# HKUST-Aerial-Robotics/FIESTA

Hardware: NVIDIA H100
Metric: esdf_voxel_updates_per_s (higher is better)
Workload: dtype int32+f64

## Files before the change

fiesta_b200/csrc/fb_exact.cu:

```cuda
#include <cub/cub.cuh>
#include <stdio.h>
#include <stdlib.h>
#include <algorithm>
#include <chrono>
#include "fb_common.cuh"
#include "fb_exact.h"

#define XNONE 0xffffffffu
#define XMB_NONE 0xffffffffffffffffull

__device__ __forceinline__ void x_coords(const FbGeom &g, uint32_t ii, int &x, int &y, int &z) {
  z = ii % (unsigned)g.pz; const unsigned xy = ii / (unsigned)g.pz; y = xy % (unsigned)g.gy; x = xy / (unsigned)g.gy;
}
__device__ __forceinline__ unsigned x_d2(int x, int y, int z, uint32_t c) {
  int ox, oy, oz; fb_unpack(c, ox, oy, oz); ox -= x; oy -= y; oz -= z;
  return (unsigned)(ox * ox + oy * oy + oz * oz);
}
__device__ __forceinline__ unsigned x_dist_of(int x, int y, int z, uint32_t c) { return c < 2u ? 0xffffffffu : x_d2(x, y, z, c); }

__global__ void k_x_flag_exist(const uint32_t *list, unsigned n, const double *occ, double l_occ, uint8_t *flags, int want) {
  const unsigned i = blockIdx.x * blockDim.x + threadIdx.x;
  if (i < n) flags[i] = ((occ[list[i]] > l_occ) ? 1 : 0) == want;
}
__global__ void k_x_apply_seed(FbGeom g, const uint32_t *E, unsigned n, uint32_t *cobs, unsigned long long *LS, unsigned long long t0) {
// ... 61 lines not shown

static inline unsigned nblk(size_t n, unsigned t = 256) { return (unsigned)((n + t - 1) / t); }

static int x_select(FbExact *X, const uint32_t *in, const uint8_t *flags, uint32_t *out, unsigned n, unsigned *count, cudaStream_t s) {
  *count = 0;
  if (n == 0) return FIESTA_OK;
  size_t bytes = 0;
  CK(cub::DeviceSelect::Flagged(nullptr, bytes, in, flags, out, X->d_count.p, (int)n, s));
  CK(X->cub_tmp.grow(bytes, s));
  CK(cub::DeviceSelect::Flagged(X->cub_tmp.p, bytes, in, flags, out, X->d_count.p, (int)n, s));
  CK(cudaMemcpyAsync(X->h_count, X->d_count, 4, cudaMemcpyDeviceToHost, s));
  CK(cudaStreamSynchronize(s));
  *count = *X->h_count;
  return FIESTA_OK;
}
static int x_sort_pairs(FbExact *X, const unsigned long long *kin, unsigned long long *kout, const uint32_t *vin, uint32_t *vout, unsigned n, cudaStream_t s,
                        int key_bits = 64) {
  size_t bytes = 0;
  CK(cub::DeviceRadixSort::SortPairs(nullptr, bytes, kin, kout, vin, vout, (int)n, 0, key_bits, s));
  CK(X->cub_tmp.grow(bytes, s));
  CK(cub::DeviceRadixSort::SortPairs(X->cub_tmp.p, bytes, kin, kout, vin, vout, (int)n, 0, key_bits, s));
  return FIESTA_OK;
}
int fb_exact_init(FbExact *X, const FbGeom &g, int device, cudaStream_t s) {
  const size_t P = (size_t)g.ptotal;
  CK(fb_xrelax_init());
  X->relax_blocks = fb_xrelax_blocks(device);
  if (X->relax_blocks <= 0 || X->relax_blocks > FB_X_MAX_BLOCKS) { fb_set_error("exact mode init: k_x_relax does not fit on this device"); return FIESTA_ERR_CUDA; }
  CK(X->MB.alloc(P)); CK(X->LS.alloc(P)); CK(X->tkey.alloc(P));
  CK(X->touched.alloc(P));
  CK(X->SUM.alloc(P)); CK(X->SUMg.alloc(P)); CK(cudaMemsetAsync(X->SUMg, 0, P * 4, s));
  CK(X->emask.alloc(P));
  CK(X->wstamp.alloc(P)); CK(cudaMemsetAsync(X->wstamp, 0, P * 4, s));
  for (int k = 0; k < 3; ++k) { CK(X->W[k].alloc(P)); CK(X->F[k].alloc(P)); }
  for (int k = 0; k < 2; ++k) CK(X->E[k].alloc(P));
  X->dense_min = 16384u;
  if (const char *e = getenv("FIESTA_X_DENSE")) { long v = atol(e); if (v >= 0 && v <= (1 << 24)) X->dense_min = (unsigned)v; }
  X->small_max = FB_X_SMALL_DEFAULT;
  if (const char *e = getenv("FIESTA_X_SMALL")) { long v = atol(e); if (v >= 0 && v <= 65536) X->small_max = (unsigned)v; }
  CK(X->slotc.alloc(((size_t)X->small_max + 1) * 32));
  const size_t c0 = P / 8 > (1u << 20) ? P / 8 : (1u << 20);
  for (FbDevBuf<unsigned long long> *b : {&X->k1, &X->k2, &X->k1b, &X->k2b}) CK(b->grow(c0, s));
  for (FbDevBuf<uint32_t> *b : {&X->dv, &X->idx[0], &X->idx[1], &X->deps, &X->nc[0], &X->nc[1], &X->sel}) CK(b->grow(c0, s));
  CK(X->flags.grow(c0, s)); CK(X->flags2.grow(c0, s));
  CK(X->cub_tmp.grow(c0 * 16 + (64u << 20), s));
  CK(X->d_ctl.alloc(1)); CK(cudaMemsetAsync(X->d_ctl, 0, sizeof(FbXCtl), s));
  CK(X->h_ctl.alloc(1));
  CK(X->d_count.alloc(4)); CK(X->d_flag.alloc(4));
  CK(X->h_count.alloc(4));
  CK(cudaMemsetAsync(X->d_count, 0, 16, s)); CK(cudaMemsetAsync(X->d_flag, 0, 16, s));
  k_x_fill64<<<FB_SMS * 8, 256, 0, s>>>(X->MB, P, XMB_NONE);
  CK(cudaMemsetAsync(X->tkey, 0, P * 8, s));
  CK(cudaMemsetAsync(X->LS, 0, P * 8, s));
  X->tclock = 1; X->key_base = 0; X->key_epoch = 1; X->key_hi = 1ull << FB_KEY_BITS; X->gen_id = 0; X->wclock = 0; X->sclock = 0;
  CK(cudaGetLastError());
  return FIESTA_OK;
}

int fb_exact_queue_crossings(FbExact *X, const unsigned long long *ins_key, const uint32_t *ins_vox, const unsigned long long *del_key,
                             const uint32_t *del_vox, FbDevBuf<uint32_t> &ins, unsigned *n_ins, FbDevBuf<uint32_t> &del, unsigned *n_del,
                             cudaStream_t s, int *launches) {
  int r;
  CK(cudaMemcpyAsync(X->h_count, X->d_count, 8, cudaMemcpyDeviceToHost, s));
  CK(cudaStreamSynchronize(s));
  const unsigned ni = X->h_count[0], nd = X->h_count[1];
  CK(ins.grow((size_t)*n_ins + ni, s, *n_ins));
  CK(del.grow((size_t)*n_del + nd, s, *n_del));
  CK(X->k1b.grow(ni > nd ? ni : nd, s));
  if (ni) { if ((r = x_sort_pairs(X, ins_key, X->k1b, ins_vox, ins + *n_ins, ni, s, FB_KEY_BITS))) return r; *n_ins += ni; *launches += 1; }
  if (nd) { if ((r = x_sort_pairs(X, del_key, X->k1b, del_vox, del + *n_del, nd, s, FB_KEY_BITS))) return r; *n_del += nd; *launches += 1; }
// ... 77 lines not shown
        } else {
          k_x_iota<<<nblk(ndep), 256, 0, s>>>(X->idx[0], ndep);
          if ((r = x_sort_pairs(X, X->k2, X->k2b, X->idx[0], X->idx[1], ndep, s))) return r;
          k_x_gather64<<<nblk(ndep), 256, 0, s>>>(X->k1, X->idx[1], ndep, X->k1b);
          if ((r = x_sort_pairs(X, X->k1b, X->k2b, X->idx[1], X->idx[0], ndep, s))) return r;
          k_x_gather32<<<nblk(ndep), 256, 0, s>>>(X->dv, X->idx[0], ndep, X->deps);
          *launches += 5;
        }
        CK(X->flags2.grow(ndep, s));
        k_x_set_ord<<<nblk(ndep), 256, 0, s>>>(X->deps, ndep, scratch, X->nc[0], X->flags2);
        *launches += 1;
        ndep_run = ndep; ls_deps = X->tclock;
        X->tclock += ndep;
      }
    }
  }
  st->generations = 0;
  if (xdbg) { cudaStreamSynchronize(s); fprintf(stderr, "[x] seeds+deletes %.2f ms (reseed rounds %u, dependants %u)\n", ms(t_begin, now()), st->reseed_rounds, st->dependants); }
  if (nE || ndep_run) {
    if (xdbg && !X->d_dbg) CK(X->d_dbg.alloc(FB_X_DBG_WORDS));
    if (xdbg) CK(cudaMemsetAsync(X->d_dbg, 0, FB_X_DBG_WORDS * 8, s));
    if (X->sclock > 0xf0000000u) { CK(cudaMemsetAsync(X->SUMg, 0, P * 4, s)); X->sclock = 0; }
    if (X->gen_id > 0xf0000000u) X->gen_id = 0;
    if (X->wclock > 0xf0000000u) { CK(cudaMemsetAsync(X->wstamp, 0, P * 4, s)); X->wclock = 0; }
    FbXCtl *h = X->h_ctl;
    memset(h, 0, sizeof(*h));
    h->gen_id = X->gen_id; h->wclock = X->wclock; h->tclock = X->tclock; h->sclock = X->sclock;
    CK(cudaMemcpyAsync(X->d_ctl, h, sizeof(FbXCtl), cudaMemcpyHostToDevice, s));
    CK(fb_xrelax_launch(X, g, cobs, nE, X->deps, ndep_run, scratch, X->nc[0], X->flags2, occbits, ls_deps, xdbg ? X->d_dbg.p : nullptr, s));
    if (ndep_run) k_x_unset<<<nblk(ndep_run), 256, 0, s>>>(X->deps, ndep_run, scratch);
    CK(cudaMemcpyAsync(h, X->d_ctl, sizeof(FbXCtl), cudaMemcpyDeviceToHost, s));
    CK(cudaStreamSynchronize(s));
    *launches += 1;
    if (h->err) { fb_set_error(h->err == 1u ? "exact mode: generation with more than 2^27 entries" : "exact mode: behaviour fixpoint did not converge"); return FIESTA_ERR_CUDA; }
    X->gen_id = h->gen_id; X->wclock = h->wclock; X->tclock = h->tclock; X->sclock = h->sclock;
    st->generations = h->generations; st->reseed_rounds = h->reseed_rounds; st->eval_rounds = h->rounds; st->dense_rounds = h->dense_rounds;
    st->voxels_changed = h->voxels_changed; st->expansions = h->expansions;
    if (xdbg) {
      static unsigned long long hd[FB_X_DBG_WORDS];
      static double cyc_per_us = 0;
      if (cyc_per_us == 0) { int dev = 0, khz = 0; CK(cudaGetDevice(&dev)); CK(cudaDeviceGetAttribute(&khz, cudaDevAttrClockRate, dev)); cyc_per_us = khz / 1000.0; }
      CK(cudaMemcpy(hd, X->d_dbg, sizeof(hd), cudaMemcpyDeviceToHost));
      static const char *cat[14] = {"S", "round1", "rounds", "dense", "commit", "apply", "s.round1", "s.rounds", "s.commit", "s.apply", "top", "empty-barrier", "reseed.rounds", "reseed.assemble"};
      fprintf(stderr, "[x] reseed rounds %u; phases (us, count):", st->reseed_rounds);
      for (int c = 0; c < 14; ++c) fprintf(stderr, " %s %.0f/%llu", cat[c], hd[3 * 1024 + 2 * c] / cyc_per_us, hd[3 * 1024 + 2 * c + 1]);
      fprintf(stderr, "\n");
      { double wm = 0; for (int q = 0; q < 4096; ++q) wm += hd[3 * 1024 + 32 + 1024 + q] / cyc_per_us; fprintf(stderr, "[x] sum over rounds of the longest per-CTA work time: %.0f us (the rest of round1+rounds+dense+s.round1+s.rounds is barrier + skew)\n", wm); }
      for (int gq = 0; gq < 2; ++gq) { fprintf(stderr, "[x] gen %d work lists:", gq); for (int r = 0; r < 512 && hd[3 * 1024 + 32 + gq * 512 + r]; ++r) fprintf(stderr, " %llu", hd[3 * 1024 + 32 + gq * 512 + r]); fprintf(stderr, "\n"); }
      fprintf(stderr, "[x] work-list entries: evaluated %llu refreshed %llu reseeded %llu\n", hd[3 * 1024 + 2 * 14], hd[3 * 1024 + 2 * 14 + 1], hd[3 * 1024 + 2 * 15]);
      fprintf(stderr, "[x] gens %u rounds %u dense %u deps %u nE0 %u |", st->generations, st->eval_rounds, st->dense_rounds, st->dependants, nE);
      for (unsigned q = 0; q < st->generations && q < 1024; ++q) fprintf(stderr, " %llu/%llu/%.1fus", hd[3 * q], hd[3 * q + 1], hd[3 * q + 2] / cyc_per_us);
      fprintf(stderr, "\n");
    }
  }
  X->scratch_clean = scratch_ok;
  return FIESTA_OK;
}
```

fiesta_b200/csrc/fb_exact.h:

```cpp
#pragma once
#include "fb_common.cuh"

#define FB_X_MAX_BLOCKS 256
#define FB_X_SMALL_DEFAULT 32768u
#define FB_X_DBG_WORDS (3 * 1024 + 32 + 2 * 512 + 4096)

struct FbExactStats {
  unsigned long long expansions;
  unsigned long long voxels_changed;
  unsigned generations, eval_rounds, dense_rounds, reseed_rounds, dependants;
};

struct FbXCtl {
  unsigned bar, err;
  unsigned sclock, pad1;
  unsigned nW[3], nF[3];
  unsigned gen_id, wclock;
  unsigned generations, rounds, dense_rounds, reseed_rounds;
  unsigned long long tclock, expansions, voxels_changed;
  unsigned partial[FB_X_MAX_BLOCKS];
};

struct FbExact {
  FbDevBuf<unsigned long long> MB;
  FbDevBuf<unsigned long long> LS;
  FbDevBuf<unsigned long long> tkey;
  FbDevBuf<uint32_t> touched;
  unsigned long long tclock = 0;
  unsigned long long key_base = 0;
  unsigned long long key_hi = 0;
  unsigned key_epoch = 0;
  FbDevBuf<unsigned> d_count, d_flag;
  FbHostBuf<unsigned> h_count;
  bool scratch_clean = false;
  FbDevBuf<uint4> SUM;
  FbDevBuf<uint32_t> SUMg;
  unsigned gen_id = 0, wclock = 0, sclock = 0;
  FbDevBuf<uint32_t> emask;
  FbDevBuf<uint32_t> W[3], F[3];
  FbDevBuf<uint32_t> wstamp;
  FbDevBuf<uint32_t> slotc;
  unsigned dense_min = 0;
  unsigned small_max = 0;
  FbDevBuf<FbXCtl> d_ctl;
  FbHostBuf<FbXCtl> h_ctl;
  FbDevBuf<unsigned long long> d_dbg;
  int relax_blocks = 0;
  FbDevBuf<uint32_t> E[2], sel;
  FbDevBuf<unsigned long long> k1, k2, k1b, k2b;
  FbDevBuf<uint32_t> dv, idx[2], deps, nc[2];
  FbDevBuf<uint8_t> flags, flags2;
  FbDevBuf<char> cub_tmp;
};

int fb_exact_init(FbExact *X, const FbGeom &g, int device, cudaStream_t s);
int fb_exact_queue_crossings(FbExact *X, const unsigned long long *ins_key, const uint32_t *ins_vox, const unsigned long long *del_key,
                             const uint32_t *del_vox, FbDevBuf<uint32_t> &ins, unsigned *n_ins, FbDevBuf<uint32_t> &del, unsigned *n_del,
                             cudaStream_t s, int *launches);
int fb_exact_next_epoch(FbExact *X, const FbGeom &g, cudaStream_t s);
int fb_exact_update_esdf(FbExact *X, const FbGeom &g, uint32_t *cobs, uint32_t *scratch, const double *occ, const uint32_t *occbits, double l_occ,
                         const uint32_t *ins, unsigned n_ins, const uint32_t *del, unsigned n_del, cudaStream_t s, FbExactStats *st, int *launches);
cudaError_t fb_xrelax_init();
int fb_xrelax_blocks(int device);
cudaError_t fb_xrelax_launch(FbExact *X, const FbGeom &g, uint32_t *cobs, unsigned nE0, const uint32_t *deps, unsigned ndep, uint32_t *ord, uint32_t *nc, uint8_t *nk,
                             const uint32_t *occbits, unsigned long long ls_deps, unsigned long long *dbg, cudaStream_t s);
```

fiesta_b200/csrc/fb_xrelax.cu:

```cuda
#include <stdio.h>
#include "fb_common.cuh"
#include "fb_exact.h"
#include "fb_divmagic.h"

#define XT 1024
#define XW (XT / 32)
#define XNONE 0xffffffffu
#define X_DEAD 0ull
#define X_PULL 1ull
#define X_PUSH 2ull
#define XMB_NONE 0xffffffffffffffffull
#define X_NOFF 129
#define X_MAX_ROUNDS 4000000u
#define XGB 8
#define XRC 8
#define XDBG_GENS 1024
#define XDBG_PHASE (3 * XDBG_GENS)
#define XDBG_ROUNDS (XDBG_PHASE + 32)
#define XDBG_WMAX (XDBG_ROUNDS + 1024)

static __constant__ int x_dirs[24][3] = {
    {-1, 0, 0}, {1, 0, 0}, {0, -1, 0}, {0, 1, 0}, {0, 0, -1}, {0, 0, 1},
    {-1, -1, 0}, {1, 1, 0}, {0, -1, -1}, {0, 1, 1}, {-1, 0, -1}, {1, 0, 1},
    {-1, 1, 0}, {1, -1, 0}, {0, -1, 1}, {0, 1, -1}, {1, 0, -1}, {-1, 0, 1},
    {-2, 0, 0}, {2, 0, 0}, {0, -2, 0}, {0, 2, 0}, {0, 0, -2}, {0, 0, 2}};
static __constant__ int x_off_c[X_NOFF];

__device__ __forceinline__ unsigned x_vi(const FbGeom &g, int x, int y, int z) { return (unsigned)((x * g.gy + y) * g.pz + z); }
__device__ __forceinline__ bool x_in_grid(const FbGeom &g, int x, int y, int z) {
  return (unsigned)x < (unsigned)g.gx && (unsigned)y < (unsigned)g.gy && (unsigned)z < (unsigned)g.gz;
}
__device__ __forceinline__ bool x_in_range(const FbGeom &g, int x, int y, int z) {
  return (unsigned)(x - g.min_vec[0]) <= (unsigned)(g.max_vec[0] - g.min_vec[0]) && (unsigned)(y - g.min_vec[1]) <= (unsigned)(g.max_vec[1] - g.min_vec[1]) &&
         (unsigned)(z - g.min_vec[2]) <= (unsigned)(g.max_vec[2] - g.min_vec[2]);
}
__device__ __forceinline__ int x_dc(int j, int k) {
  const int D[24][3] = {{-1, 0, 0}, {1, 0, 0}, {0, -1, 0}, {0, 1, 0}, {0, 0, -1}, {0, 0, 1}, {-1, -1, 0}, {1, 1, 0}, {0, -1, -1}, {0, 1, 1}, {-1, 0, -1}, {1, 0, 1},
                        {-1, 1, 0}, {1, -1, 0}, {0, -1, 1}, {0, 1, -1}, {1, 0, -1}, {-1, 0, 1}, {-2, 0, 0}, {2, 0, 0}, {0, -2, 0}, {0, 2, 0}, {0, 0, -2}, {0, 0, 2}};
  return D[j][k];
}
__device__ __forceinline__ unsigned long long x_writer_word(const FbGeom &g, const unsigned long long *MB, unsigned v, int x, int y, int z, int j, bool inr) {
  const int dx = x_dc(j, 0), dy = x_dc(j, 1), dz = x_dc(j, 2);
  const bool ok = inr && (dx == 0 || (unsigned)(x - dx) < (unsigned)g.gx) && (dy == 0 || (unsigned)(y - dy) < (unsigned)g.gy) &&
                  (dz == 0 || (unsigned)(z - dz) < (unsigned)g.gz);
  return ok ? __ldcg(&MB[v - (unsigned)((dx * g.gy + dy) * g.pz + dz)]) : XMB_NONE;
}

struct XShared {
  int off[X_NOFF];
  int dir[32];
  unsigned char slot[25 * 24];
  unsigned char self[32];
  unsigned red[XW], red2[XW];
  unsigned base, total;
};

__device__ __forceinline__ unsigned x_d2(int x, int y, int z, uint32_t c) {
  int ox, oy, oz; fb_unpack(c, ox, oy, oz); ox -= x; oy -= y; oz -= z;
  return (unsigned)(ox * ox + oy * oy + oz * oz);
}
__device__ __forceinline__ unsigned x_dist_of(int x, int y, int z, uint32_t c) { return c < 2u ? 0xffffffffu : x_d2(x, y, z, c); }
__device__ __forceinline__ unsigned long long x_mb(unsigned par, unsigned i, unsigned long long kind, uint32_t code) {
  return ((unsigned long long)(par & 1u) << 63) | ((unsigned long long)i << 33) | (kind << 31) | (unsigned long long)(code & FB_CODE_MASK);
}
__device__ __forceinline__ unsigned x_mb_idx(unsigned long long w) { return (unsigned)(w >> 33) & 0x7ffffffu; }
__device__ __forceinline__ unsigned x_mb_par(unsigned long long w) { return (unsigned)(w >> 63); }
__device__ __forceinline__ unsigned long long x_mb_kind(unsigned long long w) { return (w >> 31) & 3ull; }
__device__ __forceinline__ uint32_t x_mb_code(unsigned long long w) { return (uint32_t)(w & FB_CODE_MASK); }

struct XState { unsigned d; uint32_t c; unsigned ts; };
struct XNb { unsigned long long w[X_NOFF + 3]; uint32_t c[28]; };

template <bool WANT_FIRST>
__device__ __forceinline__ XState x_gather(const FbGeom &g, const uint32_t *cobs, const unsigned long long *MB, int x, int y, int z, unsigned T,
                                           unsigned &first, uint32_t &snap) {
  XState s;
  const unsigned v = x_vi(g, x, y, z);
  const bool inr = x_in_range(g, x, y, z);
  unsigned long long w[XGB];
  const uint32_t snap_raw = __ldcg(&cobs[v]);
  const unsigned long long wown = __ldcg(&MB[v]);
#pragma unroll
  for (int j = 0; j < XGB; ++j) w[j] = x_writer_word(g, MB, v, x, y, z, j, inr);
  snap = snap_raw & FB_CODE_MASK;
  s.c = snap; s.d = (snap_raw & FB_DINF) ? 0xffffffffu : x_dist_of(x, y, z, s.c); s.ts = XNONE;
  first = XNONE;
  const unsigned d0 = s.d;
// ... 53 lines not shown
  return v;
}
__device__ __forceinline__ void x_gsync(unsigned *bar, unsigned &target) {
  __syncthreads();
  if (threadIdx.x == 0) {
    target += gridDim.x;
    asm volatile("red.release.gpu.global.add.u32 [%0], %1;" ::"l"(bar), "r"(1u) : "memory");
    while (x_ld_acquire(bar) < target) { }
  }
  __syncthreads();
}

struct XArgs {
  FbGeom g;
  uint32_t *cobs;
  unsigned long long *MB, *LS;
  uint4 *SUM;
  uint32_t *SUMg;
  uint32_t *E[2];
  uint32_t *emask;
  uint32_t *W[3], *F[3];
  uint32_t *wstamp;
  uint32_t *slotc;
  FbXCtl *ctl;
  unsigned nE0, small_max, dense_min;
  const uint32_t *deps; unsigned ndep;
  uint32_t *ord;
  uint32_t *nc;
  uint8_t *nk;
  const uint32_t *occbits;
  unsigned long long ls_deps;
  unsigned long long *dbg;
  unsigned div_pz_m, div_pz_s, div_gy_m, div_gy_s;
};
__device__ __forceinline__ unsigned x_div(unsigned n, unsigned m, unsigned s) { return m ? (__umulhi(n, m) >> s) : n; }
__device__ __forceinline__ void x_coords(const XArgs &a, uint32_t ii, int &x, int &y, int &z) {
  const unsigned xy = x_div(ii, a.div_pz_m, a.div_pz_s);
  z = (int)(ii - xy * (unsigned)a.g.pz);
  const unsigned xx = x_div(xy, a.div_gy_m, a.div_gy_s);
  y = (int)(xy - xx * (unsigned)a.g.gy);
  x = (int)xx;
}

__device__ __forceinline__ void x_unpack_off(int o, int &dx, int &dy, int &dz) { dx = (o & 15) - 4; dy = ((o >> 4) & 15) - 4; dz = ((o >> 8) & 15) - 4; }

__device__ __forceinline__ void x_claim_summaries(const XArgs &a, const XShared &sh, unsigned lane, int x, int y, int z, unsigned sclock) {
  if (lane >= 25u) return;
  int dx, dy, dz; x_unpack_off(sh.dir[lane], dx, dy, dz);
  const int nx = x + dx, ny = y + dy, nz = z + dz;
  if (!x_in_grid(a.g, nx, ny, nz) || !(lane == 24u || x_in_range(a.g, nx, ny, nz))) return;
  const unsigned n = x_vi(a.g, nx, ny, nz);
  if (__ldcg(&a.SUMg[n]) != sclock && atomicExch(&a.SUMg[n], sclock) != sclock) x_summarize(a.g, a.cobs, a.MB, a.SUM, nx, ny, nz);
}

__device__ __forceinline__ void x_refresh_summaries(const XArgs &a, const XShared &sh, unsigned lane, unsigned i, uint32_t p, int x, int y, int z) {
  unsigned long long w = 0;
  if (lane == 0) w = __ldcg(&a.MB[p]);
  w = __shfl_sync(0xffffffffu, w, 0);
  if (lane >= 25u) return;
  int dx, dy, dz; x_unpack_off(sh.dir[lane], dx, dy, dz);
  const int nx = x + dx, ny = y + dy, nz = z + dz;
  if (!x_in_grid(a.g, nx, ny, nz) || !(lane == 24u || x_in_range(a.g, nx, ny, nz))) return;
  const uint4 u = __ldcg(&a.SUM[x_vi(a.g, nx, ny, nz)]);
  if (u.w == FB_UNKNOWN) return;
  const unsigned ts = i * 32u + lane;
  bool redo = u.x == ts || u.y == ts;
// ... 182 lines not shown
  for (int t = 0; t < 5; ++t) if ((pm >> t) & 1u) a.W[out][base++] = j[t];
}

__device__ __forceinline__ unsigned x_block_scan(XShared &sh, unsigned c, unsigned lane, unsigned wid, unsigned &total) {
  unsigned incl = c;
#pragma unroll
  for (int o = 1; o < 32; o <<= 1) { const unsigned t = __shfl_up_sync(0xffffffffu, incl, o); if ((int)lane >= o) incl += t; }
  __syncthreads();
  if (lane == 31) sh.red[wid] = incl;
  __syncthreads();
  const unsigned v = sh.red[lane]; unsigned s = v;
#pragma unroll
  for (int o = 1; o < 32; o <<= 1) { const unsigned t = __shfl_up_sync(0xffffffffu, s, o); if ((int)lane >= o) s += t; }
  total = __shfl_sync(0xffffffffu, s, 31);
  return __shfl_sync(0xffffffffu, s - v, (int)wid) + incl - c;
}

__device__ __forceinline__ unsigned x_warp_append_n(unsigned *counter, unsigned n, unsigned lane) {
  const unsigned act = __activemask(), below = (1u << lane) - 1u;
  unsigned pre = 0, total = 0;
#pragma unroll
  for (int bit = 0; bit < 4; ++bit) {
    const unsigned m = __ballot_sync(act, (n >> bit) & 1u);
    pre += (unsigned)__popc(m & below) << bit;
    total += (unsigned)__popc(m) << bit;
  }
  if (total == 0u) return 0u;
  const int leader = __ffs(act) - 1;
  unsigned base = 0;
  if ((int)lane == leader) base = atomicAdd(counter, total);
  return __shfl_sync(act, base, leader) + pre;
}

__device__ __forceinline__ uint32_t x_reseed_eval(const XArgs &a, unsigned i, int x, int y, int z, unsigned &kc) {
  const FbGeom &g = a.g;
  kc = 24u;
  for (int k = 0; k < 24; ++k) {
    const int nx = x + x_dirs[k][0], ny = y + x_dirs[k][1], nz = z + x_dirs[k][2];
    if (!x_in_range(g, nx, ny, nz) || !x_in_grid(g, nx, ny, nz)) continue;
    const unsigned nv = x_vi(g, nx, ny, nz);
    const unsigned o = __ldcg(&a.ord[nv]);
    uint32_t c;
    if (o != XNONE) { if (o < i) c = __ldcg(&a.nc[o]); else continue; }
    else c = __ldcg(&a.cobs[nv]) & FB_CODE_MASK;
    if (c >= 2u) {
      int ox, oy, oz; fb_unpack(c, ox, oy, oz);
      const unsigned oi = x_vi(g, ox, oy, oz);
      if ((__ldg(&a.occbits[oi >> 5]) >> (oi & 31)) & 1u) { kc = (unsigned)k; return c; }
    }
  }
  return FB_INF;
}

extern __shared__ __align__(16) unsigned char x_dyn_smem[];

__global__ void __launch_bounds__(XT, 1) k_x_relax(const XArgs a) {
  __shared__ XShared sh;
  const FbGeom &g = a.g;
  FbXCtl *ctl = a.ctl;
  const unsigned tid = threadIdx.x, lane = tid & 31u, wid = tid >> 5;
  const unsigned G = gridDim.x, b = blockIdx.x;
  const unsigned gtid = b * XT + tid, gthreads = G * XT;
  const unsigned gwarp = gtid >> 5, gwarps = gthreads >> 5;
  for (unsigned k = tid; k < X_NOFF; k += XT) sh.off[k] = x_off_c[k];
  if (tid < 32) sh.self[tid] = 0;
  if (tid < 32) sh.dir[tid] = tid < 24 ? ((x_dirs[tid][0] + 4) | ((x_dirs[tid][1] + 4) << 4) | ((x_dirs[tid][2] + 4) << 8)) : (4 | (4 << 4) | (4 << 8));
  __syncthreads();
  for (unsigned q = tid; q < 25u * 24u + 25u; q += XT) {
    const unsigned t = q < 600u ? q / 24u : q - 600u, k = q < 600u ? q % 24u : 24u;
    int tx, ty, tz, kx = 0, ky = 0, kz = 0; x_unpack_off(sh.dir[t], tx, ty, tz);
    if (k < 24u) x_unpack_off(sh.dir[k], kx, ky, kz);
    const int code = (tx - kx + 4) | ((ty - ky + 4) << 4) | ((tz - kz + 4) << 8);
    unsigned found = 0;
    for (unsigned o = 0; o < X_NOFF; ++o) if (sh.off[o] == code) found = o;
    if (q < 600u) sh.slot[q] = (unsigned char)found; else sh.self[t] = (unsigned char)found;
  }
  __syncthreads();
  XNb &stg = reinterpret_cast<XNb *>(x_dyn_smem)[wid];

  unsigned nE = a.nE0, bar_target = 0;
  int cur = 0;
  unsigned gen = ctl->gen_id, wclock = ctl->wclock;
  unsigned long long tclock = ctl->tclock;
  unsigned generations = 0, rounds_total = 0, dense_total = 0;
  unsigned long long changed_total = 0;
  if (a.dbg) {
    const long long t0 = clock64();
    for (int q = 0; q < 32; ++q) x_gsync(&ctl->bar, bar_target);
    if (gtid == 0) a.dbg[XDBG_PHASE + 2 * 11] = (unsigned long long)(clock64() - t0) / 32ull;
  }
  long long t_ph = a.dbg ? clock64() : 0;
#define X_LAP(cat) do { if (a.dbg && gtid == 0) { const long long t_now = clock64(); a.dbg[XDBG_PHASE + 2 * (cat)] += (unsigned long long)(t_now - t_ph); a.dbg[XDBG_PHASE + 2 * (cat) + 1] += 1ull; t_ph = t_now; } } while (0)
  unsigned reseed_rounds = 0;
  if (a.ndep) {
    for (unsigned r = 1;; ++r) {
      const unsigned in = r % 3u, out = (r + 1u) % 3u, zz = (r + 2u) % 3u;
      const unsigned nw = r == 1u ? a.ndep : __ldcg(&ctl->nW[in]);
      if (gtid == 0) ctl->nW[zz] = 0;
// ... 97 lines not shown
    for (unsigned i0 = lo; i0 < hi; i0 += XT) {
      const unsigned i = i0 + tid;
      uint32_t c = FB_INF, v = 0;
      if (i < hi) {
        c = __ldcg(&a.nc[i]); v = __ldcg(&a.deps[i]);
        a.cobs[v] = c;
        a.LS[v] = a.ls_deps + i;
      }
      unsigned ctot;
      const unsigned pos = x_block_scan(sh, (i < hi && c >= 2u) ? 1u : 0u, lane, wid, ctot);
      if (i < hi && c >= 2u) a.E[0][run + pos] = v;
      run += ctot;
    }
    nE += sh.total;
    x_gsync(&ctl->bar, bar_target);
    X_LAP(13);
  }
  bool big = nE > a.small_max;

  ++gen;
  unsigned sclock = ctl->sclock;
  for (unsigned i = gtid; i < nE; i += gthreads) {
    const uint32_t v = __ldcg(&a.E[0][i]);
    a.MB[v] = x_mb(gen, i, X_PUSH, __ldcg(&a.cobs[v]) & FB_CODE_MASK);
  }
  x_gsync(&ctl->bar, bar_target);

  while (nE) {
    const long long t_gen = a.dbg ? clock64() : 0;
    X_LAP(10);
    ++generations;
    const uint32_t *E = a.E[cur];
    unsigned rounds = 0;
    if (big) {
      ++sclock;
      for (unsigned i = gwarp; i < nE; i += gwarps) { int x, y, z; x_coords(a, __ldcg(&E[i]), x, y, z); x_claim_summaries(a, sh, lane, x, y, z, sclock); }
      x_gsync(&ctl->bar, bar_target);
      X_LAP(0);
    }
    for (unsigned r = 1;; ++r) {
      const unsigned in = r % 3u, out = (r + 1u) % 3u, zz = (r + 2u) % 3u;
      const unsigned nw = r == 1u ? nE : __ldcg(&ctl->nW[in]);
      const unsigned nf = (big && r > 1u) ? __ldcg(&ctl->nF[in]) : 0u;
      if (gtid == 0) { ctl->nW[zz] = 0; ctl->nF[zz] = 0; }
      if (r > 1u && nw == 0u && nf == 0u) break;
      if (r > X_MAX_ROUNDS) { if (gtid == 0) ctl->err = 2u; break; }
      if (a.dbg && gtid == 0) { a.dbg[XDBG_PHASE + 2 * 14] += nw; a.dbg[XDBG_PHASE + 2 * 14 + 1] += nf; }
      ++rounds; ++wclock;
      const bool dense = big && r > 1u && nw > a.dense_min;
      if (dense) {
        ++dense_total;
        if (nf < nE / 4u) {
          for (unsigned q = gwarp; q < nf; q += gwarps) {
            const unsigned i = __ldcg(&a.F[in][q]);
            const uint32_t p = __ldcg(&E[i]);
            int x, y, z; x_coords(a, p, x, y, z);
            x_refresh_summaries(a, sh, lane, i, p, x, y, z);
          }
        } else {
          ++sclock;
          for (unsigned i = gwarp; i < nE; i += gwarps) { int x, y, z; x_coords(a, __ldcg(&E[i]), x, y, z); x_claim_summaries(a, sh, lane, x, y, z, sclock); }
        }
        x_gsync(&ctl->bar, bar_target);
      }
      const bool use_sum = big && (r == 1u || dense);
      const unsigned nref = (big && !dense) ? nf : 0u;
      const uint32_t *wl = a.W[in];
      const long long t_w0 = a.dbg ? clock64() : 0;
      for (unsigned q = gwarp; q < nw + nref; q += gwarps) {
        if (q >= nw) {
          const unsigned i = __ldcg(&a.F[in][q - nw]);
          const uint32_t p = __ldcg(&E[i]);
          int x, y, z; x_coords(a, p, x, y, z);
          x_refresh_summaries(a, sh, lane, i, p, x, y, z);
          continue;
        }
        const unsigned i = r == 1u ? q : __ldcg(&wl[q]);
        const uint32_t p = __ldcg(&E[i]);
        int x, y, z; x_coords(a, p, x, y, z);
        if (!use_sum) {
          x_stage(a, sh, stg, lane, x, y, z);
          const unsigned long long old = stg.w[0], nw2 = x_eval_nb(a, sh, stg, lane, gen, i, x, y, z);
          if (nw2 == old) continue;
          if (lane == 0) {
            a.MB[p] = nw2;
            if (big) a.F[out][atomicAdd(&ctl->nF[out], 1u)] = i;
          }
          x_list_affected_nb(a, stg, lane, i, (x_mb_kind(old) == X_PUSH || x_mb_kind(nw2) == X_PUSH) ? (unsigned)X_NOFF : 25u, wclock, out);
          continue;
        }
        unsigned long long old = 0;
        if (lane == 0) old = __ldcg(&a.MB[p]);
        const unsigned long long nb = x_eval<true>(a, sh, lane, gen, i, p, x, y, z);
        old = __shfl_sync(0xffffffffu, old, 0);
        if (nb == old) continue;
        if (lane == 0) {
          a.MB[p] = nb;
          if (big) a.F[out][atomicAdd(&ctl->nF[out], 1u)] = i;
        }
        x_list_affected(a, sh, lane, i, x, y, z, (x_mb_kind(old) == X_PUSH || x_mb_kind(nb) == X_PUSH) ? (unsigned)X_NOFF : 25u, wclock, out);
      }
      if (a.dbg) { __syncthreads(); if (tid == 0) atomicMax(&a.dbg[XDBG_WMAX + ((rounds_total + rounds) & 4095u)], (unsigned long long)(clock64() - t_w0)); }
      x_gsync(&ctl->bar, bar_target);
      X_LAP(big ? (r == 1u ? 1 : (dense ? 3 : 2)) : (r == 1u ? 6 : 7));
      if (a.dbg && gtid == 0 && generations <= 2u && rounds <= 512u) a.dbg[XDBG_ROUNDS + (generations - 1u) * 512u + (rounds - 1u)] = nw;
    }
    rounds_total += rounds;
    if (rounds > X_MAX_ROUNDS) break;

    const unsigned per = (nE + G - 1u) / G;
    const unsigned lo = min(nE, b * per), hi = min(nE, lo + per);
    unsigned wcount = 0, wlive = 0;
    for (unsigned i = lo + wid; i < hi; i += XW) {
      const uint32_t p = __ldcg(&E[i]);
      int x, y, z; x_coords(a, p, x, y, z);
      unsigned long long w = 0;
      if (!big) { x_stage(a, sh, stg, lane, x, y, z); w = stg.w[0]; }
      else { if (lane == 0) w = __ldcg(&a.MB[p]); w = __shfl_sync(0xffffffffu, w, 0); }
      const unsigned long long kind = x_mb_kind(w);
      bool win = false;
      if ((kind == X_PUSH && lane < 24) || (kind == X_PULL && lane == 24)) {
        int dx, dy, dz; x_unpack_off(sh.dir[lane], dx, dy, dz);
        const int nx = x + dx, ny = y + dy, nz = z + dz;
        if (x_in_grid(g, nx, ny, nz) && (lane == 24 || x_in_range(g, nx, ny, nz))) {
          const unsigned ts = i * 32u + lane;
          if (big) win = __ldcg(&a.SUM[x_vi(g, nx, ny, nz)]).y == ts;
          else {
            uint32_t snap;
            const XState f = x_state_nb(g, sh, stg, lane, nx, ny, nz, XNONE, snap);
            win = f.ts == ts;
            if (win) a.slotc[ts] = f.c;
          }
        }
      }
      const unsigned m = __ballot_sync(0xffffffffu, win);
      if (lane == 0) { a.emask[i] = m; wcount += __popc(m); wlive += kind != X_DEAD ? 1u : 0u; }
    }
    if (lane == 0) { sh.red[wid] = wcount; sh.red2[wid] = wlive; }
    __syncthreads();
    if (wid == 0) {
      unsigned c = sh.red[lane], l = sh.red2[lane];
// ... 16 lines not shown
    const unsigned n2 = sh.total;
    const bool big2 = n2 > a.small_max;
    uint32_t *En = a.E[cur ^ 1];
    unsigned run = sh.base;
    for (unsigned i0 = lo; i0 < hi; i0 += XT) {
      const unsigned i = i0 + tid;
      const uint32_t m = i < hi ? __ldcg(&a.emask[i]) : 0u;
      if (i < hi) {
        const uint32_t p = __ldcg(&E[i]);
        const unsigned long long w = __ldcg(&a.MB[p]);
        if (w != XMB_NONE && x_mb_par(w) == (gen & 1u)) atomicCAS(&a.MB[p], w, XMB_NONE);
      }
      unsigned ctot;
      unsigned r = run + x_block_scan(sh, (unsigned)__popc(m), lane, wid, ctot);
      if (m) {
        const uint32_t p = __ldcg(&E[i]);
        int x, y, z; x_coords(a, p, x, y, z);
        uint32_t me = m;
        while (me) {
          const int k = __ffs(me) - 1; me &= me - 1u;
          int dx, dy, dz; x_unpack_off(sh.dir[k], dx, dy, dz);
          const uint32_t v = (uint32_t)x_vi(g, x + dx, y + dy, z + dz);
          const unsigned ts = i * 32u + (unsigned)k;
          const uint32_t code = big ? __ldcg(&a.SUM[v]).z : __ldcg(&a.slotc[ts]);
          a.cobs[v] = code;
          a.LS[v] = tclock + ts;
          En[r] = v;
          a.MB[v] = x_mb(gen + 1u, r, X_PUSH, code);
          ++r;
        }
      }
      run += ctot;
    }
    if (a.dbg && gtid == 0 && generations <= 1024u) { a.dbg[3 * (generations - 1u)] = nE; a.dbg[3 * (generations - 1u) + 1] = rounds; a.dbg[3 * (generations - 1u) + 2] = (unsigned long long)(clock64() - t_gen); }
    tclock += (unsigned long long)nE * 32ull + 1ull;
    changed_total += n2;
    if (n2 >= (1u << 27)) { if (gtid == 0) ctl->err = 1u; break; }
    const bool was_big = big;
    nE = n2; cur ^= 1; big = big2; ++gen;
    x_gsync(&ctl->bar, bar_target);
    X_LAP(was_big ? 5 : 9);
  }
  if (gtid == 0) {
    ctl->gen_id = gen; ctl->wclock = wclock; ctl->tclock = tclock; ctl->sclock = sclock;
    ctl->generations = generations; ctl->reseed_rounds = reseed_rounds; ctl->rounds = rounds_total; ctl->dense_rounds = dense_total; ctl->voxels_changed = changed_total;
  }
}

static bool g_off_ready = false;
cudaError_t fb_xrelax_init() {
  if (g_off_ready) return cudaSuccess;
  static const int D[24][3] = {
      {-1, 0, 0}, {1, 0, 0}, {0, -1, 0}, {0, 1, 0}, {0, 0, -1}, {0, 0, 1},
      {-1, -1, 0}, {1, 1, 0}, {0, -1, -1}, {0, 1, 1}, {-1, 0, -1}, {1, 0, 1},
      {-1, 1, 0}, {1, -1, 0}, {0, -1, 1}, {0, 1, -1}, {1, 0, -1}, {-1, 0, 1},
      {-2, 0, 0}, {2, 0, 0}, {0, -2, 0}, {0, 2, 0}, {0, 0, -2}, {0, 0, 2}};
  int off[1024], n = 0;
  for (int p = -1; p < 24; ++p)
    for (int q = -1; q < 24; ++q) {
      int o[3];
      for (int k = 0; k < 3; ++k) o[k] = (p < 0 ? 0 : D[p][k]) + (q < 0 ? 0 : D[q][k]);
      const int code = (o[0] + 4) | ((o[1] + 4) << 4) | ((o[2] + 4) << 8);
      bool dup = false;
      for (int j = 0; j < n; ++j) dup = dup || off[j] == code;
      if (!dup) off[n++] = code;
    }
  if (n != X_NOFF) return cudaErrorUnknown;
  cudaError_t e = cudaMemcpyToSymbol(x_off_c, off, sizeof(int) * X_NOFF);
  if (e == cudaSuccess) g_off_ready = true;
  return e;
}

int fb_xrelax_blocks(int device) {
  int per_sm = 0, sms = 0;
  if (cudaOccupancyMaxActiveBlocksPerMultiprocessor(&per_sm, k_x_relax, XT, sizeof(XNb) * XW) != cudaSuccess || per_sm < 1) return -1;
  if (cudaDeviceGetAttribute(&sms, cudaDevAttrMultiProcessorCount, device) != cudaSuccess) return -1;
  return sms;
}

cudaError_t fb_xrelax_launch(FbExact *X, const FbGeom &g, uint32_t *cobs, unsigned nE0, const uint32_t *deps, unsigned ndep, uint32_t *ord, uint32_t *nc, uint8_t *nk,
                             const uint32_t *occbits, unsigned long long ls_deps, unsigned long long *dbg, cudaStream_t s) {
  XArgs a;
  a.deps = deps; a.ndep = ndep; a.ord = ord; a.nc = nc; a.nk = nk; a.occbits = occbits; a.ls_deps = ls_deps;
  fb_div_make((unsigned)g.pz, a.div_pz_m, a.div_pz_s);
  fb_div_make((unsigned)g.gy, a.div_gy_m, a.div_gy_s);
  a.g = g;
  if (a.g.max_vec[0] < a.g.min_vec[0] || a.g.max_vec[1] < a.g.min_vec[1] || a.g.max_vec[2] < a.g.min_vec[2])
    for (int k = 0; k < 3; ++k) a.g.min_vec[k] = a.g.max_vec[k] = 0x3fffffff;
  a.cobs = cobs; a.MB = X->MB; a.LS = X->LS; a.SUM = X->SUM; a.SUMg = X->SUMg;
  a.E[0] = X->E[0]; a.E[1] = X->E[1]; a.emask = X->emask;
  for (int k = 0; k < 3; ++k) { a.W[k] = X->W[k]; a.F[k] = X->F[k]; }
  a.wstamp = X->wstamp; a.slotc = X->slotc; a.ctl = X->d_ctl; a.nE0 = nE0; a.small_max = X->small_max; a.dense_min = X->dense_min; a.dbg = dbg;
  void *args[] = {(void *)&a};
  return cudaLaunchCooperativeKernel((void *)k_x_relax, dim3(X->relax_blocks), dim3(XT), args, sizeof(XNb) * XW, s);
}
```

Before: 119.2 million.

## Replace barrier-synchronised sparse relaxation rounds with an asynchronous global work queue

For big generations, once the work list falls below the dense threshold, the remaining bulk-synchronous rounds are replaced by a persistent device-wide ring-buffer queue. Warps pop voxels, re-evaluate them, and push changed neighbours without grid barriers, using wstamp to dedupe and to flag a voxel as dirty for re-evaluation. Summaries are then refreshed once for all changed voxels. This aims to remove the per-round grid-sync and skew cost of long sparse tails, at the price of atomic contention, spin-waiting, and a timeout abort path.

```diff
diff --git a/fiesta_b200/csrc/fb_exact.cu b/fiesta_b200/csrc/fb_exact.cu
--- a/fiesta_b200/csrc/fb_exact.cu
+++ b/fiesta_b200/csrc/fb_exact.cu
@@ -117,10 +117,11 @@
   CK(X->SUM.alloc(P)); CK(X->SUMg.alloc(P)); CK(cudaMemsetAsync(X->SUMg, 0, P * 4, s));
   CK(X->emask.alloc(P));
   CK(X->wstamp.alloc(P)); CK(cudaMemsetAsync(X->wstamp, 0, P * 4, s));
-  for (int k = 0; k < 3; ++k) { CK(X->W[k].alloc(P)); CK(X->F[k].alloc(P)); }
+  for (int k = 0; k < 3; ++k) { CK(X->W[k].alloc(P)); CK(X->F[k].alloc(P)); CK(cudaMemsetAsync(X->W[k], 0, P * 4, s)); }
   for (int k = 0; k < 2; ++k) CK(X->E[k].alloc(P));
   X->dense_min = 16384u;
   if (const char *e = getenv("FIESTA_X_DENSE")) { long v = atol(e); if (v >= 0 && v <= (1 << 24)) X->dense_min = (unsigned)v; }
+  if (const char *e = getenv("FIESTA_X_ASYNC")) X->async = atol(e) != 0;
   X->small_max = FB_X_SMALL_DEFAULT;
   if (const char *e = getenv("FIESTA_X_SMALL")) { long v = atol(e); if (v >= 0 && v <= 65536) X->small_max = (unsigned)v; }
   CK(X->slotc.alloc(((size_t)X->small_max + 1) * 32));
@@ -264,7 +265,16 @@
     CK(cudaMemcpyAsync(h, X->d_ctl, sizeof(FbXCtl), cudaMemcpyDeviceToHost, s));
     CK(cudaStreamSynchronize(s));
     *launches += 1;
-    if (h->err) { fb_set_error(h->err == 1u ? "exact mode: generation with more than 2^27 entries" : "exact mode: behaviour fixpoint did not converge"); return FIESTA_ERR_CUDA; }
+    if (h->err) {
+      if (h->err == 3u) {
+        for (int k = 0; k < 3; ++k) CK(cudaMemsetAsync(X->W[k], 0, P * 4, s));
+        CK(cudaMemsetAsync(X->wstamp, 0, P * 4, s));
+        X->wclock = 0;
+      }
+      fb_set_error(h->err == 1u ? "exact mode: generation with more than 2^27 entries"
+                   : h->err == 3u ? "exact mode: a wait of the asynchronous work queue exceeded its bound" : "exact mode: behaviour fixpoint did not converge");
+      return FIESTA_ERR_CUDA;
+    }
     X->gen_id = h->gen_id; X->wclock = h->wclock; X->tclock = h->tclock; X->sclock = h->sclock;
     st->generations = h->generations; st->reseed_rounds = h->reseed_rounds; st->eval_rounds = h->rounds; st->dense_rounds = h->dense_rounds;
     st->voxels_changed = h->voxels_changed; st->expansions = h->expansions;
@@ -273,15 +283,26 @@
       static double cyc_per_us = 0;
       if (cyc_per_us == 0) { int dev = 0, khz = 0; CK(cudaGetDevice(&dev)); CK(cudaDeviceGetAttribute(&khz, cudaDevAttrClockRate, dev)); cyc_per_us = khz / 1000.0; }
       CK(cudaMemcpy(hd, X->d_dbg, sizeof(hd), cudaMemcpyDeviceToHost));
-      static const char *cat[14] = {"S", "round1", "rounds", "dense", "commit", "apply", "s.round1", "s.rounds", "s.commit", "s.apply", "top", "empty-barrier", "reseed.rounds", "reseed.assemble"};
+      static const char *cat[19] = {"S", "round1", "rounds", "dense", "commit", "apply", "s.round1", "s.rounds", "s.commit", "s.apply", "top", "empty-barrier",
+                                    "reseed.rounds", "reseed.assemble", "", "", "async", "", "refresh"};
       fprintf(stderr, "[x] reseed rounds %u; phases (us, count):", st->reseed_rounds);
-      for (int c = 0; c < 14; ++c) fprintf(stderr, " %s %.0f/%llu", cat[c], hd[3 * 1024 + 2 * c] / cyc_per_us, hd[3 * 1024 + 2 * c + 1]);
+      for (int c = 0; c < 19; ++c)
+        if (*cat[c]) fprintf(stderr, " %s %.0f/%llu", cat[c], hd[FB_XDBG_PHASE + 2 * c] / cyc_per_us, hd[FB_XDBG_PHASE + 2 * c + 1]);
       fprintf(stderr, "\n");
-      { double wm = 0; for (int q = 0; q < 4096; ++q) wm += hd[3 * 1024 + 32 + 1024 + q] / cyc_per_us; fprintf(stderr, "[x] sum over rounds of the longest per-CTA work time: %.0f us (the rest of round1+rounds+dense+s.round1+s.rounds is barrier + skew)\n", wm); }
-      for (int gq = 0; gq < 2; ++gq) { fprintf(stderr, "[x] gen %d work lists:", gq); for (int r = 0; r < 512 && hd[3 * 1024 + 32 + gq * 512 + r]; ++r) fprintf(stderr, " %llu", hd[3 * 1024 + 32 + gq * 512 + r]); fprintf(stderr, "\n"); }
-      fprintf(stderr, "[x] work-list entries: evaluated %llu refreshed %llu reseeded %llu\n", hd[3 * 1024 + 2 * 14], hd[3 * 1024 + 2 * 14 + 1], hd[3 * 1024 + 2 * 15]);
+      fprintf(stderr, "[x] round work (summed longest CTA work time us / summed list length):");
+      for (int c : {1, 2, 3, 6, 7}) fprintf(stderr, " %s %.0f/%llu", cat[c], hd[FB_XDBG_WORK + 2 * c] / cyc_per_us, hd[FB_XDBG_WORK + 2 * c + 1]);
+      fprintf(stderr, "\n");
+      for (int h = 0; h < 2; ++h) {
+        fprintf(stderr, "[x] list-length histogram %s (log2 bucket=rounds):", h ? "s.rounds" : "rounds");
+        for (int b = 0; b < 32; ++b) if (hd[FB_XDBG_NWH + 32 * h + b]) fprintf(stderr, " %d=%llu", b, hd[FB_XDBG_NWH + 32 * h + b]);
+        fprintf(stderr, "\n");
+      }
+      fprintf(stderr, "[x] async: evaluations %llu dirty %llu pushes %llu spin %.0f us\n", hd[FB_XDBG_Q + 0], hd[FB_XDBG_Q + 1], hd[FB_XDBG_Q + 2],
+              hd[FB_XDBG_Q + 3] / cyc_per_us);
+      for (int gq = 0; gq < 2; ++gq) { fprintf(stderr, "[x] gen %d work lists:", gq); for (int r = 0; r < 512 && hd[FB_XDBG_ROUNDS + gq * 512 + r]; ++r) fprintf(stderr, " %llu", hd[FB_XDBG_ROUNDS + gq * 512 + r]); fprintf(stderr, "\n"); }
+      fprintf(stderr, "[x] work-list entries: evaluated %llu refreshed %llu reseeded %llu\n", hd[FB_XDBG_PHASE + 2 * 14], hd[FB_XDBG_PHASE + 2 * 14 + 1], hd[FB_XDBG_PHASE + 2 * 15]);
       fprintf(stderr, "[x] gens %u rounds %u dense %u deps %u nE0 %u |", st->generations, st->eval_rounds, st->dense_rounds, st->dependants, nE);
-      for (unsigned q = 0; q < st->generations && q < 1024; ++q) fprintf(stderr, " %llu/%llu/%.1fus", hd[3 * q], hd[3 * q + 1], hd[3 * q + 2] / cyc_per_us);
+      for (unsigned q = 0; q < st->generations && q < FB_XDBG_GENS; ++q) fprintf(stderr, " %llu/%llu/%.1fus", hd[3 * q], hd[3 * q + 1], hd[3 * q + 2] / cyc_per_us);
       fprintf(stderr, "\n");
     }
   }
diff --git a/fiesta_b200/csrc/fb_exact.h b/fiesta_b200/csrc/fb_exact.h
--- a/fiesta_b200/csrc/fb_exact.h
+++ b/fiesta_b200/csrc/fb_exact.h
@@ -3,7 +3,16 @@
 
 #define FB_X_MAX_BLOCKS 256
 #define FB_X_SMALL_DEFAULT 32768u
-#define FB_X_DBG_WORDS (3 * 1024 + 32 + 2 * 512 + 4096)
+#define FB_XDBG_GENS 1024
+#define FB_XDBG_NCAT 24
+#define FB_XDBG_NQ 8
+#define FB_XDBG_PHASE (3 * FB_XDBG_GENS)
+#define FB_XDBG_ROUNDS (FB_XDBG_PHASE + 2 * FB_XDBG_NCAT)
+#define FB_XDBG_WMAX (FB_XDBG_ROUNDS + 2 * 512)
+#define FB_XDBG_WORK (FB_XDBG_WMAX + 4096)
+#define FB_XDBG_NWH (FB_XDBG_WORK + 2 * FB_XDBG_NCAT)
+#define FB_XDBG_Q (FB_XDBG_NWH + 2 * 32)
+#define FB_X_DBG_WORDS (FB_XDBG_Q + FB_XDBG_NQ)
 
 struct FbExactStats {
   unsigned long long expansions;
@@ -19,6 +28,9 @@
   unsigned generations, rounds, dense_rounds, reseed_rounds;
   unsigned long long tclock, expansions, voxels_changed;
   unsigned partial[FB_X_MAX_BLOCKS];
+  alignas(128) unsigned long long qtail;
+  alignas(128) unsigned qhead;
+  alignas(128) unsigned qdone;
 };
 
 struct FbExact {
@@ -42,6 +54,7 @@
   FbDevBuf<uint32_t> slotc;
   unsigned dense_min = 0;
   unsigned small_max = 0;
+  bool async = true;
   FbDevBuf<FbXCtl> d_ctl;
   FbHostBuf<FbXCtl> h_ctl;
   FbDevBuf<unsigned long long> d_dbg;
diff --git a/fiesta_b200/csrc/fb_xrelax.cu b/fiesta_b200/csrc/fb_xrelax.cu
--- a/fiesta_b200/csrc/fb_xrelax.cu
+++ b/fiesta_b200/csrc/fb_xrelax.cu
@@ -14,10 +14,9 @@
 #define X_MAX_ROUNDS 4000000u
 #define XGB 8
 #define XRC 8
-#define XDBG_GENS 1024
-#define XDBG_PHASE (3 * XDBG_GENS)
-#define XDBG_ROUNDS (XDBG_PHASE + 32)
-#define XDBG_WMAX (XDBG_ROUNDS + 1024)
+#define XDBG_PHASE FB_XDBG_PHASE
+#define XDBG_ROUNDS FB_XDBG_ROUNDS
+#define XDBG_WMAX FB_XDBG_WMAX
 
 static __constant__ int x_dirs[24][3] = {
     {-1, 0, 0}, {1, 0, 0}, {0, -1, 0}, {0, 1, 0}, {0, 0, -1}, {0, 0, 1},
@@ -53,6 +52,7 @@
   unsigned char self[32];
   unsigned red[XW], red2[XW];
   unsigned base, total;
+  unsigned qdone;
 };
 
 __device__ __forceinline__ unsigned x_d2(int x, int y, int z, uint32_t c) {
@@ -172,6 +172,7 @@
   unsigned long long ls_deps;
   unsigned long long *dbg;
   unsigned div_pz_m, div_pz_s, div_gy_m, div_gy_s;
+  unsigned async_on;
 };
 __device__ __forceinline__ unsigned x_div(unsigned n, unsigned m, unsigned s) { return m ? (__umulhi(n, m) >> s) : n; }
 __device__ __forceinline__ void x_coords(const XArgs &a, uint32_t ii, int &x, int &y, int &z) {
@@ -420,6 +421,149 @@
   return __shfl_sync(act, base, leader) + pre;
 }
 
+#define X_Q_FULL 0x80000000u
+#define X_Q_WAIT_NS 2000000000ull
+__device__ __forceinline__ unsigned x_ld_relaxed(const unsigned *p) {
+  unsigned v;
+  asm volatile("ld.relaxed.gpu.global.u32 %0, [%1];" : "=r"(v) : "l"(p) : "memory");
+  return v;
+}
+__device__ __forceinline__ unsigned long long x_globaltimer() {
+  unsigned long long t;
+  asm volatile("mov.u64 %0, %%globaltimer;" : "=l"(t));
+  return t;
+}
+__device__ __forceinline__ void x_q_abort(const XArgs &a) {
+  atomicCAS(&a.ctl->err, 0u, 3u);
+  atomicExch(&a.ctl->qdone, 1u);
+}
+__device__ __forceinline__ unsigned x_q_count(const XArgs &a, unsigned long long delta) {
+  const unsigned long long old = atomicAdd(&a.ctl->qtail, delta);
+  if ((unsigned)((old + delta) >> 32) == 0u) atomicExch(&a.ctl->qdone, 1u);
+  return (unsigned)old;
+}
+__device__ __forceinline__ void x_q_put(const XArgs &a, XShared &sh, uint32_t *ring, unsigned cap, unsigned idx, unsigned e) {
+  unsigned *slot = &ring[idx % cap];
+  const volatile unsigned *done = &sh.qdone;
+  unsigned cur = x_ld_relaxed(slot);
+  const unsigned long long t0 = x_globaltimer();
+  for (unsigned it = 0;; ++it) {
+    if (!(cur & X_Q_FULL)) {
+      const unsigned o = atomicCAS(slot, cur, e | X_Q_FULL);
+      if (o == cur) return;
+      cur = o;
+      continue;
+    }
+    if (*done) return;
+    if ((it & 15u) == 15u) {
+      if (x_ld_acquire(&a.ctl->qdone)) { sh.qdone = 1u; return; }
+      if (x_globaltimer() - t0 > X_Q_WAIT_NS) { x_q_abort(a); sh.qdone = 1u; return; }
+    }
+    __nanosleep(64);
+    cur = x_ld_relaxed(slot);
+  }
+}
+__device__ __forceinline__ unsigned x_q_take(const XArgs &a, XShared &sh, uint32_t *ring, unsigned cap, unsigned &h) {
+  if (h == XNONE) h = atomicAdd(&a.ctl->qhead, 1u);
+  unsigned *slot = &ring[h % cap];
+  const volatile unsigned *done = &sh.qdone;
+  const long long c0 = a.dbg ? clock64() : 0;
+  unsigned long long t0 = 0;
+  unsigned ns = 32;
+  for (unsigned it = 0;; ++it) {
+    if (x_ld_relaxed(slot) & X_Q_FULL) {
+      const unsigned v = atomicExch(slot, 0u);
+      if (v & X_Q_FULL) { h = XNONE; if (a.dbg) atomicAdd(&a.dbg[FB_XDBG_Q + 3], (unsigned long long)(clock64() - c0)); return v & ~X_Q_FULL; }
+    }
+    if (*done) break;
+    if ((it & 15u) == 15u) {
+      if (x_ld_acquire(&a.ctl->qdone)) { sh.qdone = 1u; break; }
+      const unsigned long long t = x_globaltimer();
+      if (t0 == 0) t0 = t;
+      else if (t - t0 > X_Q_WAIT_NS) { x_q_abort(a); sh.qdone = 1u; break; }
+    }
+    __nanosleep(ns);
+    ns = ns < 256u ? 2u * ns : 256u;
+  }
+  if (a.dbg) atomicAdd(&a.dbg[FB_XDBG_Q + 3], (unsigned long long)(clock64() - c0));
+  return XNONE;
+}
+__device__ __forceinline__ unsigned x_q_list(const XArgs &a, XShared &sh, const XNb &nb, uint32_t *ring, unsigned cap, unsigned lane, unsigned i, unsigned nof, unsigned A) {
+  unsigned j[5], st[5];
+#pragma unroll
+  for (int t = 0; t < 5; ++t) {
+    const unsigned o = lane + 32u * (unsigned)t;
+    const unsigned long long w = o < nof ? nb.w[o] : XMB_NONE;
+    j[t] = w != XMB_NONE ? x_mb_idx(w) : 0u;
+    st[t] = (w != XMB_NONE && j[t] > i) ? x_ld_relaxed(&a.wstamp[j[t]]) : A + 1u;
+  }
+  unsigned pm = 0;
+#pragma unroll
+  for (int t = 0; t < 5; ++t)
+    if (st[t] != A + 1u && atomicMax(&a.wstamp[j[t]], A + 1u) < A) pm |= 1u << t;
+  const unsigned cnt = (unsigned)__popc(pm);
+  unsigned incl = cnt;
+#pragma unroll
+  for (int o = 1; o < 32; o <<= 1) { const unsigned v = __shfl_up_sync(0xffffffffu, incl, o); if ((int)lane >= o) incl += v; }
+  const unsigned total = __shfl_sync(0xffffffffu, incl, 31);
+  if (total == 0u) return 0u;
+  unsigned base = 0;
+  if (lane == 0) base = x_q_count(a, (unsigned long long)total * 0x100000001ull);
+  base = __shfl_sync(0xffffffffu, base, 0) + incl - cnt;
+#pragma unroll
+  for (int t = 0; t < 5; ++t) if ((pm >> t) & 1u) x_q_put(a, sh, ring, cap, base++, j[t]);
+  return total;
+}
+__device__ void x_async(const XArgs &a, XShared &sh, XNb &stg, unsigned lane, unsigned gwarp, unsigned gwarps, const uint32_t *E, unsigned nE,
+                        const uint32_t *wl, unsigned nw, uint32_t *ring, unsigned gen, unsigned A, unsigned fout) {
+  for (unsigned q0 = gwarp * 32u; q0 < nw; q0 += gwarps * 32u) {
+    const unsigned q = q0 + lane;
+    const unsigned e = q < nw ? __ldcg(&wl[q]) : 0u;
+    const bool push = q < nw && atomicMax(&a.wstamp[e], A + 1u) < A;
+    const unsigned pm = __ballot_sync(0xffffffffu, push), cnt = (unsigned)__popc(pm);
+    if (cnt == 0u) continue;
+    unsigned base = 0;
+    if (lane == 0) base = x_q_count(a, (unsigned long long)cnt * 0x100000001ull);
+    base = __shfl_sync(0xffffffffu, base, 0);
+    if (push) x_q_put(a, sh, ring, nE, base + (unsigned)__popc(pm & ((1u << lane) - 1u)), e);
+    if (a.dbg && lane == 0) atomicAdd(&a.dbg[FB_XDBG_Q + 2], (unsigned long long)cnt);
+  }
+  if (lane == 0) x_q_count(a, 0ull - (1ull << 32));
+  unsigned h = XNONE;
+  for (;;) {
+    unsigned i = 0;
+    if (lane == 0) i = x_q_take(a, sh, ring, nE, h);
+    i = __shfl_sync(0xffffffffu, i, 0);
+    if (i == XNONE) break;
+    const uint32_t p = __ldcg(&E[i]);
+    int x, y, z; x_coords(a, p, x, y, z);
+    for (;;) {
+      if (a.dbg && lane == 0) atomicAdd(&a.dbg[FB_XDBG_Q + 0], 1ull);
+      if (lane == 0) atomicExch(&a.wstamp[i], A);
+      __syncwarp();
+      __threadfence();
+      x_stage(a, sh, stg, lane, x, y, z);
+      const unsigned long long old = stg.w[0], nw2 = x_eval_nb(a, sh, stg, lane, gen, i, x, y, z);
+      if (nw2 != old) {
+        if (lane == 0) {
+          a.MB[p] = nw2;
+          const unsigned f = atomicAdd(&a.ctl->nF[fout], 1u);
+          if (f < (unsigned)a.g.ptotal) a.F[fout][f] = i;
+        }
+        __syncwarp();
+        __threadfence();
+        const unsigned np = x_q_list(a, sh, stg, ring, nE, lane, i, (x_mb_kind(old) == X_PUSH || x_mb_kind(nw2) == X_PUSH) ? (unsigned)X_NOFF : 25u, A);
+        if (a.dbg && lane == 0 && np) atomicAdd(&a.dbg[FB_XDBG_Q + 2], (unsigned long long)np);
+      }
+      unsigned again = 0;
+      if (lane == 0) again = atomicCAS(&a.wstamp[i], A, A - 1u) != A ? 1u : 0u;
+      if (!__shfl_sync(0xffffffffu, again, 0)) break;
+      if (a.dbg && lane == 0) atomicAdd(&a.dbg[FB_XDBG_Q + 1], 1ull);
+    }
+    if (lane == 0) x_q_count(a, 0ull - (1ull << 32));
+  }
+}
+
 __device__ __forceinline__ uint32_t x_reseed_eval(const XArgs &a, unsigned i, int x, int y, int z, unsigned &kc) {
   const FbGeom &g = a.g;
   kc = 24u;
@@ -452,6 +596,8 @@
   const unsigned gwarp = gtid >> 5, gwarps = gthreads >> 5;
   for (unsigned k = tid; k < X_NOFF; k += XT) sh.off[k] = x_off_c[k];
   if (tid < 32) sh.self[tid] = 0;
+  if (tid == 0) sh.qdone = 0u;
+  if (gtid == 0) a.ctl->qtail = (unsigned long long)gwarps << 32;
   if (tid < 32) sh.dir[tid] = tid < 24 ? ((x_dirs[tid][0] + 4) | ((x_dirs[tid][1] + 4) << 4) | ((x_dirs[tid][2] + 4) << 8)) : (4 | (4 << 4) | (4 << 8));
   __syncthreads();
   for (unsigned q = tid; q < 25u * 24u + 25u; q += XT) {
@@ -615,6 +761,7 @@
     ++generations;
     const uint32_t *E = a.E[cur];
     unsigned rounds = 0;
+    bool aborted = false;
     if (big) {
       ++sclock;
       for (unsigned i = gwarp; i < nE; i += gwarps) { int x, y, z; x_coords(a, __ldcg(&E[i]), x, y, z); x_claim_summaries(a, sh, lane, x, y, z, sclock); }
@@ -629,6 +776,31 @@
       if (r > 1u && nw == 0u && nf == 0u) break;
       if (r > X_MAX_ROUNDS) { if (gtid == 0) ctl->err = 2u; break; }
       if (a.dbg && gtid == 0) { a.dbg[XDBG_PHASE + 2 * 14] += nw; a.dbg[XDBG_PHASE + 2 * 14 + 1] += nf; }
+      if (a.async_on && big && r > 1u && nw <= a.dense_min) {
+        ++rounds; wclock += 3u;
+        const unsigned A = wclock - 1u;
+        x_async(a, sh, stg, lane, gwarp, gwarps, E, nE, a.W[in], nw, a.W[out], gen, A, out);
+        x_gsync(&ctl->bar, bar_target);
+        X_LAP(16);
+        if (tid == 0) sh.qdone = 0u;
+        if (gtid == 0) { ctl->qtail = (unsigned long long)gwarps << 32; ctl->qhead = 0u; ctl->qdone = 0u; }
+        if (__ldcg(&ctl->err)) { aborted = true; break; }
+        const unsigned nfa = __ldcg(&ctl->nF[out]);
+        if (nfa > (unsigned)g.ptotal) {
+          ++sclock;
+          for (unsigned i = gwarp; i < nE; i += gwarps) { int x, y, z; x_coords(a, __ldcg(&E[i]), x, y, z); x_claim_summaries(a, sh, lane, x, y, z, sclock); }
+        } else {
+          for (unsigned q = gwarp; q < nf + nfa; q += gwarps) {
+            const unsigned i = q < nf ? __ldcg(&a.F[in][q]) : __ldcg(&a.F[out][q - nf]);
+            const uint32_t p = __ldcg(&E[i]);
+            int x, y, z; x_coords(a, p, x, y, z);
+            x_refresh_summaries(a, sh, lane, i, p, x, y, z);
+          }
+        }
+        x_gsync(&ctl->bar, bar_target);
+        X_LAP(18);
+        break;
+      }
       ++rounds; ++wclock;
       const bool dense = big && r > 1u && nw > a.dense_min;
       if (dense) {
@@ -686,10 +858,16 @@
       if (a.dbg) { __syncthreads(); if (tid == 0) atomicMax(&a.dbg[XDBG_WMAX + ((rounds_total + rounds) & 4095u)], (unsigned long long)(clock64() - t_w0)); }
       x_gsync(&ctl->bar, bar_target);
       X_LAP(big ? (r == 1u ? 1 : (dense ? 3 : 2)) : (r == 1u ? 6 : 7));
-      if (a.dbg && gtid == 0 && generations <= 2u && rounds <= 512u) a.dbg[XDBG_ROUNDS + (generations - 1u) * 512u + (rounds - 1u)] = nw;
+      if (a.dbg && gtid == 0) {
+        if (generations <= 2u && rounds <= 512u) a.dbg[XDBG_ROUNDS + (generations - 1u) * 512u + (rounds - 1u)] = nw;
+        const unsigned cat = big ? (r == 1u ? 1u : (dense ? 3u : 2u)) : (r == 1u ? 6u : 7u);
+        unsigned long long *wm = &a.dbg[XDBG_WMAX + ((rounds_total + rounds) & 4095u)];
+        a.dbg[FB_XDBG_WORK + 2 * cat] += __ldcg(wm); a.dbg[FB_XDBG_WORK + 2 * cat + 1] += nw; *wm = 0;
+        if (cat == 2u || cat == 7u) a.dbg[FB_XDBG_NWH + (cat == 7u ? 32u : 0u) + (nw ? 32u - __clz(nw) : 0u)] += 1ull;
+      }
     }
     rounds_total += rounds;
-    if (rounds > X_MAX_ROUNDS) break;
+    if (rounds > X_MAX_ROUNDS || aborted) break;
 
     const unsigned per = (nE + G - 1u) / G;
     const unsigned lo = min(nE, b * per), hi = min(nE, lo + per);
@@ -772,7 +950,7 @@
       }
       run += ctot;
     }
-    if (a.dbg && gtid == 0 && generations <= 1024u) { a.dbg[3 * (generations - 1u)] = nE; a.dbg[3 * (generations - 1u) + 1] = rounds; a.dbg[3 * (generations - 1u) + 2] = (unsigned long long)(clock64() - t_gen); }
+    if (a.dbg && gtid == 0 && generations <= FB_XDBG_GENS) { a.dbg[3 * (generations - 1u)] = nE; a.dbg[3 * (generations - 1u) + 1] = rounds; a.dbg[3 * (generations - 1u) + 2] = (unsigned long long)(clock64() - t_gen); }
     tclock += (unsigned long long)nE * 32ull + 1ull;
     changed_total += n2;
     if (n2 >= (1u << 27)) { if (gtid == 0) ctl->err = 1u; break; }
@@ -831,6 +1009,7 @@
   a.E[0] = X->E[0]; a.E[1] = X->E[1]; a.emask = X->emask;
   for (int k = 0; k < 3; ++k) { a.W[k] = X->W[k]; a.F[k] = X->F[k]; }
   a.wstamp = X->wstamp; a.slotc = X->slotc; a.ctl = X->d_ctl; a.nE0 = nE0; a.small_max = X->small_max; a.dense_min = X->dense_min; a.dbg = dbg;
+  a.async_on = X->async ? 1u : 0u;
   void *args[] = {(void *)&a};
   return cudaLaunchCooperativeKernel((void *)k_x_relax, dim3(X->relax_blocks), dim3(XT), args, sizeof(XNb) * XW, s);
 }
```

Result: faster. 126.3 million (median of 6 runs) (+6.0%).
